# invictus717/MiCo

Hardware: AMD Instinct MI355X
Metric: omni-modal samples/sec (ViT-g/14 fwd+bwd) (higher is better)
Workload: dtype fp16

## Files before the change

mico_amd/csrc/attention.hip:

```cpp
#include "common.h"
#include <type_traits>

namespace {

constexpr float NEG_BIG = -1.0e30f;

#ifndef MICO_ATTN_PRIO
#define MICO_ATTN_PRIO 0
#endif

#ifdef MICO_ATTN_PHASES
__device__ unsigned long long g_attn_phase[4096 * 8];
#define PH_DECL unsigned long long ph_t = __builtin_readcyclecounter(), ph_acc[8] = {0, 0, 0, 0, 0, 0, 0, 0}
#define PH(slot) do { const unsigned long long n_ = __builtin_readcyclecounter(); ph_acc[slot] += n_ - ph_t; ph_t = n_; } while (0)
#define PH_STORE do { const int wg_ = (blockIdx.z * gridDim.y + blockIdx.y) * gridDim.x + blockIdx.x; \
        if (lane == 0 && wave == 0 && wg_ < 4096) for (int e_ = 0; e_ < 8; ++e_) g_attn_phase[wg_ * 8 + e_] = ph_acc[e_]; } while (0)
#else
#define PH_DECL
#define PH(slot)
#define PH_STORE
#endif

template <int HDP> struct Cfg {
    static constexpr int RS = 256;
// ... 32 lines not shown
}
template <int HDP>
__device__ __forceinline__ void tile_commit(const s16x8 (&reg)[Cfg<HDP>::NCH], LDS_AS char* tile, const TileMap<HDP>& m) {
#pragma unroll
    for (int it = 0; it < Cfg<HDP>::NCH; ++it) *(LDS_AS s16x8*)(tile + m.loff[it]) = reg[it];
}

template <typename T, int HDP>
__device__ __forceinline__ void row_frags(s16x8 (&f)[Cfg<HDP>::KS], const T* base, int64_t rs, int row, int nrows, int hd,
                                          int lane) {
#pragma unroll
    for (int ks = 0; ks < Cfg<HDP>::KS; ++ks) {
        const int d = ks * 32 + (lane >> 4) * 8;
        s16x8 v = {0, 0, 0, 0, 0, 0, 0, 0};
        if (row < nrows && d < hd) v = *(const s16x8*)(base + (int64_t)row * rs + d);
        f[ks] = v;
    }
}

template <int KM> __device__ __forceinline__ int swz_key(int row) {
    return KM == 0 ? ((row & 7) << 1) : (((row & 3) << 2) | ((row >> 2) & 3));
}
template <int HDP, int KM = 0>
__device__ __forceinline__ s16x8 lds_row_frag(LDS_AS const char* tile, int r0, int ks, int lane) {
    const int row = r0 + (lane & 15), ch = ks * 4 + (lane >> 4);
    return *(LDS_AS const s16x8*)(tile + row * Cfg<HDP>::RS + ((ch ^ swz_key<KM>(row)) << 4));
}
template <int HDP, int KM = 0>
__device__ __forceinline__ s16x8 lds_tr_frag(LDS_AS const char* tile, int td, int s2, int lane) {
    const int g = lane >> 4, p = lane & 15;
    const int ch = td * 2 + ((p >> 1) & 1), half = (p & 1) * 8;
    const int r_lo = (2 * s2) * 16 + g * 4 + (p >> 2);
    const int col_b = ((ch ^ swz_key<KM>(r_lo)) << 4) + half;
    s16x4 lo = __builtin_amdgcn_ds_read_tr16_b64_v4i16((LDS_AS s16x4*)(tile + r_lo * Cfg<HDP>::RS + col_b));
    s16x4 hi = __builtin_amdgcn_ds_read_tr16_b64_v4i16((LDS_AS s16x4*)(tile + (r_lo + 16) * Cfg<HDP>::RS + col_b));
    s16x8 r;
    r[0] = lo[0]; r[1] = lo[1]; r[2] = lo[2]; r[3] = lo[3];
    r[4] = hi[0]; r[5] = hi[1]; r[6] = hi[2]; r[7] = hi[3];
    return r;
}

__device__ __forceinline__ void lds_dma16(__amdgpu_buffer_rsrc_t rsrc, unsigned lds_dst, unsigned voffset) {
    unsigned keep;
    const unsigned dst = __builtin_amdgcn_readfirstlane(lds_dst);
    asm volatile("s_mov_b32 %0, m0\n\ts_mov_b32 m0, %2\n\ts_nop 0\n\tbuffer_load_dwordx4 %1, %3, 0 offen lds\n\ts_mov_b32 m0, %0"
                 : "=&s"(keep) : "v"(voffset), "s"(dst), "s"(rsrc) : "memory");
}

__device__ __forceinline__ void* uniform_ptr(const void* ptr) {
    const unsigned long long v = (unsigned long long)ptr;
    const unsigned lo = __builtin_amdgcn_readfirstlane((unsigned)v), hi = __builtin_amdgcn_readfirstlane((unsigned)(v >> 32));
    return (void*)(((unsigned long long)hi << 32) | lo);
}

template <typename T>
__device__ __forceinline__ s16x8 pack_pair(const f32x4& a, const f32x4& b) {
    typename T16<T>::v8 v;
    v[0] = (T)a[0]; v[1] = (T)a[1]; v[2] = (T)a[2]; v[3] = (T)a[3];
    v[4] = (T)b[0]; v[5] = (T)b[1]; v[6] = (T)b[2]; v[7] = (T)b[3];
    return __builtin_bit_cast(s16x8, v);
}

__device__ __forceinline__ float group_max(float v) { return xor32_max(xor16_max(v)); }
__device__ __forceinline__ float group_sum(float v) { return xor32_sum(xor16_sum(v)); }

__device__ __forceinline__ float mask_val(const float* mask, int mode, int b, int i, int j, int Sq, int Sk) {
    if (mode == 1) return mask[(int64_t)b * Sk + j];
    if (mode == 2) return mask[((int64_t)b * Sq + i) * Sk + j];
    return 0.f;
}

template <typename T, int HDP, bool DROP, int RB, int NW = 4>
__global__ __launch_bounds__(NW * 64, 2) void attn_fwd_kernel(const T* __restrict__ q, const T* __restrict__ k,
                                                              const T* __restrict__ v, T* __restrict__ o,
                                                              float* __restrict__ lse, const mico_attn_params p) {
    using C = Cfg<HDP>;
    __shared__ __attribute__((aligned(16))) char smem[2 * C::TILE];
    LDS_AS char* kt = (LDS_AS char*)smem;
    LDS_AS char* vt = kt + C::TILE;
    const int tid = threadIdx.x, lane = tid & 63, wave = tid >> 6;
    const bool stager = NW == 4 || tid < 256;
    const int b = blockIdx.z, h = blockIdx.y, q0 = blockIdx.x * (NW * 16 * RB);
    const T* qb = q + (int64_t)b * p.q_bs + h * p.hd;
    const int kvb = p.kv_index ? p.kv_index[b] : (p.kv_batch_mod > 0 ? b % p.kv_batch_mod : b);
    const T* kb = k + (int64_t)kvb * p.k_bs + h * p.hd;
    const T* vb = v + (int64_t)kvb * p.v_bs + h * p.hd;
    const int i0 = q0 + wave * (16 * RB) + (lane & 15);
    const int g = lane >> 4;
    const bool wave_live = q0 + wave * (16 * RB) < p.Sq;

    s16x8 qf[RB][C::KS];
    f32x4 oacc[RB][C::TD];
    float m_run[RB], l_run[RB];
#pragma unroll
    for (int rb = 0; rb < RB; ++rb) {
        row_frags<T, HDP>(qf[rb], qb, p.q_rs, i0 + rb * 16, p.Sq, p.hd, lane);
#pragma unroll
        for (int t = 0; t < C::TD; ++t) oacc[rb][t] = (f32x4){0.f, 0.f, 0.f, 0.f};
        m_run[rb] = NEG_BIG;
        l_run[rb] = 0.f;
    }
    const float sc2 = p.scale * 1.4426950408889634f;

    const int nt = (p.Sk + 63) / 64;
    const TileMap<HDP> tm_a = tile_map<HDP>(p.k_rs, p.hd, tid), tm_b = tile_map<HDP>(p.v_rs, p.hd, tid);
    s16x8 kr[C::NCH], vr[C::NCH];
// ... 82 lines not shown
#pragma unroll
                    for (int tn = 0; tn < 4; ++tn)
#pragma unroll
                        for (int r = 0; r < 4; ++r)
                            s[rb][tn][r] *= drop_hash_t(h0, tb + (unsigned)(tn * 16 + r) * 0x85EBCA6Bu) >= thr ? ik : 0.f;
                } else {
#pragma unroll
                    for (int tn = 0; tn < 4; ++tn)
#pragma unroll
                        for (int r = 0; r < 4; ++r)
                            s[rb][tn][r] *= drop_mult(p.drop_seed, p.drop_site, rowbase + (t * 64 + tn * 16 + g * 4 + r), thr, ik);
                }
            }
            l_run[rb] = l_run[rb] * alpha + group_sum(lloc);
            m_run[rb] = m_new;
#pragma unroll
            for (int t2 = 0; t2 < C::TD; ++t2) oacc[rb][t2] *= alpha;
            pf[rb][0] = pack_pair<T>(s[rb][0], s[rb][1]);
            pf[rb][1] = pack_pair<T>(s[rb][2], s[rb][3]);
        }
        PH(5);
#pragma unroll
        for (int s2 = 0; s2 < 2; ++s2) {
            if (2 * s2 >= ntn || !wave_live) continue;
#pragma unroll
            for (int td = 0; td < C::TD; ++td) {
                const s16x8 a = lds_tr_frag<HDP>(vt, td, s2, lane);
#pragma unroll
                for (int rb = 0; rb < RB; ++rb) oacc[rb][td] = T16<T>::mfma(a, pf[rb][s2], oacc[rb][td]);
            }
        }
        PH(6);
    }
    PH_STORE;
#pragma unroll
    for (int rb = 0; rb < RB; ++rb) {
        const int i = i0 + rb * 16;
        if (i < p.Sq) {
            const float inv = 1.f / l_run[rb];
            T* ob = o + (int64_t)b * p.o_bs + (int64_t)i * p.o_rs + h * p.hd;
#pragma unroll
            for (int td = 0; td < C::TD; ++td) {
                const int d = td * 16 + g * 4;
                if (d < p.hd)
                    *(s16x4*)(ob + d) = pack4<T>(oacc[rb][td][0] * inv, oacc[rb][td][1] * inv, oacc[rb][td][2] * inv, oacc[rb][td][3] * inv);
            }
            if (g == 0) lse[((int64_t)b * p.H + h) * p.Sq + i] = (m_run[rb] + __log2f(l_run[rb])) * 0.6931471805599453f;
        }
    }
}

constexpr int RES_KR = 288;

template <typename T, int HDP, int RB, int NSUB, bool ALL>
__device__ __forceinline__ void res_tile_step(LDS_AS const char* ktile, LDS_AS const char* vtile, const int key0, const int lo,
                                              const int hi, const int mode, const s16x8 (&qf)[RB][Cfg<HDP>::KS],
                                              f32x4 (&oacc)[RB][Cfg<HDP>::TD], float (&m_run)[RB], float (&l_run)[RB],
                                              const int Sk, const float sc2, const int lane,
                                              const int (&rf)[Cfg<HDP>::KS], const int (&tf)[Cfg<HDP>::TD]) {
    using C = Cfg<HDP>;
    constexpr int NH = (NSUB + 1) / 2;
    const int g = lane >> 4;
    f32x4 s[RB][NH * 2];
    if (ALL) {
        s16x8 an[C::KS];
#pragma unroll
        for (int ks = 0; ks < C::KS; ++ks) an[ks] = *(LDS_AS const s16x8*)(ktile + rf[ks]);
#pragma unroll
        for (int tn = 0; tn < NH * 2; ++tn) {
#pragma unroll
            for (int rb = 0; rb < RB; ++rb) s[rb][tn] = (f32x4){0.f, 0.f, 0.f, 0.f};
            if (tn >= NSUB) continue;
            s16x8 ac[C::KS];
#pragma unroll
            for (int ks = 0; ks < C::KS; ++ks) ac[ks] = an[ks];
            if (tn + 1 < NSUB) {
#pragma unroll
                for (int ks = 0; ks < C::KS; ++ks) an[ks] = *(LDS_AS const s16x8*)(ktile + rf[ks] + (tn + 1) * 16 * C::RS);
            }
            __builtin_amdgcn_sched_barrier(0);
#pragma unroll
            for (int ks = 0; ks < C::KS; ++ks)
#pragma unroll
                for (int rb = 0; rb < RB; ++rb) s[rb][tn] = T16<T>::mfma(ac[ks], qf[rb][ks], s[rb][tn]);
            __builtin_amdgcn_sched_barrier(0);
        }
    } else {
#pragma unroll
        for (int tn = 0; tn < NH * 2; ++tn) {
#pragma unroll
            for (int rb = 0; rb < RB; ++rb) s[rb][tn] = (f32x4){0.f, 0.f, 0.f, 0.f};
            if (tn < NSUB && tn >= lo && tn < hi) {
#pragma unroll
                for (int ks = 0; ks < C::KS; ++ks) {
                    const s16x8 a = *(LDS_AS const s16x8*)(ktile + rf[ks] + tn * 16 * C::RS);
#pragma unroll
                    for (int rb = 0; rb < RB; ++rb) s[rb][tn] = T16<T>::mfma(a, qf[rb][ks], s[rb][tn]);
                }
            }
        }
    }
    s16x8 pf[RB][NH];
#pragma unroll
    for (int rb = 0; rb < RB; ++rb) {
        float mloc = NEG_BIG;
#pragma unroll
        for (int tn = 0; tn < NH * 2; ++tn) {
            if (tn >= NSUB) {
                s[rb][tn] = (f32x4){NEG_BIG, NEG_BIG, NEG_BIG, NEG_BIG};
            } else if (mode == 0 || (mode == 1 && tn < NSUB - 1)) {
                s[rb][tn] *= sc2;
                mloc = fmaxf(fmaxf(mloc, fmaxf(s[rb][tn][0], s[rb][tn][1])), fmaxf(s[rb][tn][2], s[rb][tn][3]));
            } else {
                const int lim = (ALL || (tn >= lo && tn < hi)) ? Sk - key0 - tn * 16 - g * 4 : 0;
#pragma unroll
                for (int r = 0; r < 4; ++r) {
                    const float x = r < lim ? s[rb][tn][r] * sc2 : NEG_BIG;
                    s[rb][tn][r] = x;
                    mloc = fmaxf(mloc, x);
                }
            }
        }
        const float m_new = fmaxf(m_run[rb], group_max(mloc));
        const float alpha = __builtin_amdgcn_exp2f(m_run[rb] - m_new);
        float lloc = 0.f;
#pragma unroll
        for (int tn = 0; tn < NH * 2; ++tn) {
            if (tn >= NSUB) {
                s[rb][tn] = (f32x4){0.f, 0.f, 0.f, 0.f};
            } else {
#pragma unroll
                for (int r = 0; r < 4; ++r) {
                    const float e = __builtin_amdgcn_exp2f(s[rb][tn][r] - m_new);
                    s[rb][tn][r] = e;
                    lloc += e;
                }
            }
        }
        l_run[rb] = l_run[rb] * alpha + group_sum(lloc);
        m_run[rb] = m_new;
#pragma unroll
        for (int t2 = 0; t2 < C::TD; ++t2) oacc[rb][t2] *= alpha;
#pragma unroll
        for (int s2 = 0; s2 < NH; ++s2) pf[rb][s2] = pack_pair<T>(s[rb][2 * s2], s[rb][2 * s2 + 1]);
    }
    auto vfrag = [&](int idx) -> s16x8 {
        const int s2 = idx / C::TD, td = idx - s2 * C::TD;
        const s16x4 alo = __builtin_amdgcn_ds_read_tr16_b64_v4i16((LDS_AS s16x4*)(vtile + tf[td] + s2 * 32 * C::RS));
        const s16x4 ahi = __builtin_amdgcn_ds_read_tr16_b64_v4i16((LDS_AS s16x4*)(vtile + tf[td] + s2 * 32 * C::RS + 16 * C::RS));
        return (s16x8){alo[0], alo[1], alo[2], alo[3], ahi[0], ahi[1], ahi[2], ahi[3]};
    };
    if (ALL) {
        constexpr int NF = NH * C::TD, AH = 3;
        s16x8 ring[AH];
#pragma unroll
        for (int i = 0; i < AH; ++i) ring[i] = vfrag(i);
#pragma unroll
        for (int i = 0; i < NF; ++i) {
            const s16x8 a = ring[i % AH];
            if (i + AH < NF) ring[i % AH] = vfrag(i + AH);
            __builtin_amdgcn_sched_barrier(0);
#pragma unroll
            for (int rb = 0; rb < RB; ++rb) oacc[rb][i % C::TD] = T16<T>::mfma(a, pf[rb][i / C::TD], oacc[rb][i % C::TD]);
            __builtin_amdgcn_sched_barrier(0);
        }
    } else {
#pragma unroll
        for (int s2 = 0; s2 < NH; ++s2) {
            if (2 * s2 + 1 < lo || 2 * s2 >= hi) continue;
#pragma unroll
            for (int td = 0; td < C::TD; ++td) {
                const s16x8 a = vfrag(s2 * C::TD + td);
#pragma unroll
                for (int rb = 0; rb < RB; ++rb) oacc[rb][td] = T16<T>::mfma(a, pf[rb][s2], oacc[rb][td]);
            }
        }
    }
}

#ifndef MICO_ATTN_R1
#define MICO_ATTN_R1 0
#endif
template <int HDP> struct ResCfg {
    static constexpr int NXMAX = HDP <= 96 ? 4 : 3;
    static constexpr int PST = HDP + 2;
};

template <typename T, int HDP>
__global__ __launch_bounds__(512, 1) void attn_fwd_res_kernel(const T* __restrict__ q, const T* __restrict__ k,
                                                              const T* __restrict__ v, T* __restrict__ o,
                                                              float* __restrict__ lse, const mico_attn_params p) {
    using C = Cfg<HDP>;
    using R = ResCfg<HDP>;
    constexpr int CPR = HDP / 8;
    constexpr int NLD = 256 * CPR / 512;
    __shared__ __attribute__((aligned(16))) char smem[2 * RES_KR * C::RS + 8 * R::NXMAX * R::PST * 4];
    LDS_AS char* kt = (LDS_AS char*)smem;
    LDS_AS char* vt = kt + RES_KR * C::RS;
    LDS_AS float* part = (LDS_AS float*)(vt + RES_KR * C::RS);
    const int tid = threadIdx.x, lane = tid & 63, wave = tid >> 6;
    const int g = lane >> 4;
    const float sc2 = p.scale * 1.4426950408889634f;
    const int nitems = p.B * p.H;

    for (int c = tid; c < 32 * 16; c += 512) {
        *(LDS_AS s16x8*)(kt + 256 * C::RS + c * 16) = (s16x8){0, 0, 0, 0, 0, 0, 0, 0};
        *(LDS_AS s16x8*)(vt + 256 * C::RS + c * 16) = (s16x8){0, 0, 0, 0, 0, 0, 0, 0};
    }
    const int xrow = 256 + tid / CPR, xch = tid - (tid / CPR) * CPR;
    const bool xlive = xrow < p.Sk && xch * 8 < p.hd;
    const int xoff = xrow * C::RS + ((xch ^ ((xrow & 7) << 1)) << 4);

    int rf[C::KS], tf[C::TD];
#pragma unroll
    for (int ks = 0; ks < C::KS; ++ks) rf[ks] = (lane & 15) * C::RS + (((ks * 4 + g) ^ ((lane & 7) << 1)) << 4);
    {
        const int pp = lane & 15, r8 = g * 4 + (pp >> 2);
#pragma unroll
        for (int td = 0; td < C::TD; ++td) tf[td] = r8 * C::RS + (((td * 2 + ((pp >> 1) & 1)) ^ ((r8 & 7) << 1)) << 4) + (pp & 1) * 8;
    }
    const int nst = (p.Sk + 15) >> 4;
    constexpr bool WIDE = HDP <= 64;
    const bool wide_last = WIDE && nst > 4 && (nst & 3) == 1;
    const bool r1 = MICO_ATTN_R1 && !WIDE && p.Sk > 64 && (p.Sk & 63) == 1;
    const int nstm = r1 ? nst - 1 : nst;
    const int nsteps = wide_last ? (nst >> 2) : ((nstm + 3) >> 2);
    const int nx = p.Sq - 256;
    const int xt = wave >> 1, xlo = (wave & 1) * 2;
    const int xhi = wave == 7 ? nst - 12 : min(xlo + 2, nst - 4 * xt);

    auto kv_off = [&](int it) -> unsigned {
        if (it == NLD) return xlive ? (unsigned)(xrow * p.k_rs * 2 + xch * 16) : 0xFFFFFFF0u;
        const int c = it * 512 + tid;
        const int row = c / CPR, ch = c - row * CPR;
        return (row < p.Sk && ch * 8 < p.hd) ? (unsigned)(row * p.k_rs * 2 + ch * 16) : 0xFFFFFFF0u;
    };
    const int kbytes = (int)(((int64_t)(p.Sk - 1) * p.k_rs + p.hd) * 2), vbytes = (int)(((int64_t)(p.Sk - 1) * p.v_rs + p.hd) * 2);
    const int qbytes = (int)(((int64_t)(p.Sq - 1) * p.q_rs + p.hd) * 2);
    auto q_off = [&](int rb, int ks) -> unsigned {
        const int row = (rb < 2 ? wave * 32 + rb * 16 : 256) + (lane & 15), d = ks * 32 + g * 8;
        return (row < p.Sq && d < p.hd) ? (unsigned)(row * p.q_rs * 2 + d * 2) : 0xFFFFFFF0u;
    };
    s16x8 kr[NLD + 1], vr[NLD + 1];
    auto prefetch_part = [&](int item, int part_id) {
        const int b = item / p.H, h = item - b * p.H;
        __amdgpu_buffer_rsrc_t rk = __builtin_amdgcn_make_buffer_rsrc((void*)(k + (int64_t)b * p.k_bs + h * p.hd), 0, kbytes, 0x00020000);
#pragma unroll
        for (int it = 0; it <= NLD; ++it) {
            if (it * 4 / (NLD + 1) != part_id) continue;
            kr[it] = __builtin_bit_cast(s16x8, __builtin_amdgcn_raw_buffer_load_b128(rk, kv_off(it), 0, 0));
        }
    };
    auto load_v = [&](int item) {
// ... 36 lines not shown
        }
    };
    const int nwg = gridDim.x;
    int item = (int)blockIdx.x;
    int item_step = nwg;
    if ((nwg & 7) == 0 && nitems % nwg == 0) {
        const int per_wg = nitems / nwg;
        item = ((int)(blockIdx.x & 7) * (nwg >> 3) + (int)(blockIdx.x >> 3)) * per_wg;
        item_step = 1;
    }
    const int item_end = item_step == 1 ? item + nitems / nwg : nitems;
    if (item < item_end) {
#pragma unroll
        for (int pt = 0; pt < 4; ++pt) prefetch_part(item, pt);
        load_v(item);
        load_q(item);
    }

    int prev = -1;
    PH_DECL;
    for (; item < item_end; item += item_step) {
        PH(7);
        const int b = item / p.H, h = item - b * p.H;
#if MICO_ATTN_PRIO
        if (((item ^ (wave >> 2)) & 1) != 0) __builtin_amdgcn_s_setprio(1); else __builtin_amdgcn_s_setprio(0);
#endif
        const int next = item + item_step < item_end ? item + item_step : item;
        __syncthreads();
        PH(0);
        if (nx > 0 && prev >= 0) merge(prev);
        PH(1);
#pragma unroll
        for (int it = 0; it < NLD; ++it) {
            const int c = it * 512 + tid;
            const int row = c / CPR, ch = c - row * CPR;
            const int off = row * C::RS + ((ch ^ ((row & 7) << 1)) << 4);
            *(LDS_AS s16x8*)(kt + off) = kr[it];
            *(LDS_AS s16x8*)(vt + off) = vr[it];
        }
        if (xlive) {
            *(LDS_AS s16x8*)(kt + xoff) = kr[NLD];
            *(LDS_AS s16x8*)(vt + xoff) = vr[NLD];
        }
        PH(2);
        __syncthreads();
        PH(3);
        prefetch_part(next, 0);
        PH(4);
        if (nx > 0) {
            f32x4 ox[1][C::TD];
            float mx[1] = {NEG_BIG}, lx[1] = {0.f};
#pragma unroll
            for (int t = 0; t < C::TD; ++t) ox[0][t] = (f32x4){0.f, 0.f, 0.f, 0.f};
            if (xhi > xlo)
                res_tile_step<T, HDP, 1, 5, false>(kt + xt * C::TILE, vt + xt * C::TILE, xt * 64, xlo, xhi, 2, qx, ox, mx, lx, p.Sk, sc2, lane, rf, tf);
            if ((lane & 15) < nx) {
                LDS_AS float* pr = part + (wave * R::NXMAX + (lane & 15)) * R::PST;
                if (g == 0) { pr[HDP] = mx[0]; pr[HDP + 1] = lx[0]; }
#pragma unroll
                for (int td = 0; td < C::TD; ++td)
#pragma unroll
                    for (int r = 0; r < 4; ++r) pr[td * 16 + g * 4 + r] = ox[0][td][r];
            }
        }
        prev = item;
        PH(5);
        const bool main_live = wave * 32 < p.Sq;
        const int i0 = wave * 32 + (lane & 15);
        f32x4 oacc[2][C::TD];
        float m_run[2] = {NEG_BIG, NEG_BIG}, l_run[2] = {0.f, 0.f};
#pragma unroll
        for (int t = 0; t < C::TD; ++t) {
            oacc[0][t] = (f32x4){0.f, 0.f, 0.f, 0.f};
            oacc[1][t] = (f32x4){0.f, 0.f, 0.f, 0.f};
        }
        if (r1 && main_live) {
            LDS_AS const char* krow = kt + (p.Sk - 1) * C::RS;
            LDS_AS const char* vrow = vt + (p.Sk - 1) * C::RS;
            float dot[2] = {0.f, 0.f};
#pragma unroll
            for (int ks = 0; ks < C::KS; ++ks) {
                float k8[8];
                unpack8<T>(*(LDS_AS const s16x8*)(krow + ((ks * 4 + g) << 4)), k8);
#pragma unroll
                for (int rb = 0; rb < 2; ++rb) {
                    float q8[8];
                    unpack8<T>(qf[rb][ks], q8);
#pragma unroll
                    for (int e = 0; e < 8; ++e) dot[rb] = __builtin_fmaf(q8[e], k8[e], dot[rb]);
                }
            }
#pragma unroll
            for (int rb = 0; rb < 2; ++rb) {
                m_run[rb] = group_sum(dot[rb]) * sc2;
                l_run[rb] = 1.f;
            }
#pragma unroll
            for (int td = 0; td < C::TD; ++td) {
                const f32x4 v4 = unpack4<T>(*(LDS_AS const s16x4*)(vrow + ((td * 2 + (g >> 1)) << 4) + (g & 1) * 8));
                oacc[0][td] = v4;
                oacc[1][td] = v4;
            }
        }
        auto key_step = [&](int t) {
            if (!main_live || t >= nsteps) return;
            LDS_AS const char* ktile = kt + t * C::TILE;
            LDS_AS const char* vtile = vt + t * C::TILE;
            if (WIDE && t == nsteps - 1 && wide_last) {
                res_tile_step<T, HDP, 2, 5, true>(ktile, vtile, t * 64, 0, 5, (p.Sk & 15) ? 1 : 0, qf, oacc, m_run, l_run, p.Sk, sc2, lane, rf, tf);
            } else {
                const int ntn = min(4, nstm - 4 * t);
                if (ntn == 4) res_tile_step<T, HDP, 2, 4, true>(ktile, vtile, t * 64, 0, 4, t * 64 + 64 <= p.Sk ? 0 : 1, qf, oacc, m_run, l_run, p.Sk, sc2, lane, rf, tf);
                else res_tile_step<T, HDP, 2, 4, false>(ktile, vtile, t * 64, 0, ntn, 2, qf, oacc, m_run, l_run, p.Sk, sc2, lane, rf, tf);
            }
        };
        key_step(0);
        prefetch_part(next, 1);
        key_step(1);
        prefetch_part(next, 2);
        key_step(2);
        prefetch_part(next, 3);
        key_step(3);
        key_step(4);
        load_v(next);
        load_q(next);
        PH(6);
        if (main_live) {
            static_assert(C::TD % 2 == 0, "tile pairs");
#pragma unroll
            for (int rb = 0; rb < 2; ++rb) {
                const int i = i0 + rb * 16;
                const float inv = 1.f / l_run[rb];
                T* ob = o + (int64_t)b * p.o_bs + (int64_t)i * p.o_rs + h * p.hd;
#pragma unroll
                for (int tp = 0; tp < C::TD; tp += 2) {
                    const f32x4 ta = oacc[rb][tp], tb = oacc[rb][tp + 1];
                    u32x2 a2 = {pack2_scaled<T>(ta[0], ta[1], inv), pack2_scaled<T>(ta[2], ta[3], inv)};
                    u32x2 c2 = {pack2_scaled<T>(tb[0], tb[1], inv), pack2_scaled<T>(tb[2], tb[3], inv)};
                    asm volatile("s_nop 1\n\tv_permlane16_swap_b32 %0, %1" : "+v"(a2[0]), "+v"(c2[0]));
                    asm volatile("s_nop 1\n\tv_permlane16_swap_b32 %0, %1" : "+v"(a2[1]), "+v"(c2[1]));
                    const int d = (tp + (g & 1)) * 16 + (g >> 1) * 8;
                    if (i < p.Sq && d < p.hd) *(u32x4*)(ob + d) = (u32x4){a2[0], a2[1], c2[0], c2[1]};
                }
                if (i < p.Sq && g == 0) lse[((int64_t)b * p.H + h) * p.Sq + i] = (m_run[rb] + __log2f(l_run[rb])) * 0.6931471805599453f;
            }
        }
    }
    if (nx > 0 && prev >= 0) {
        __syncthreads();
        merge(prev);
    }
#ifdef MICO_ATTN_PHASES
    if (lane == 0 && blockIdx.x < 512) for (int e_ = 0; e_ < 8; ++e_) g_attn_phase[(blockIdx.x * 8 + wave) * 8 + e_] = ph_acc[e_];
#endif
}

template <typename T, int HDP, bool DROP>
__global__ __launch_bounds__(256, 2) void attn_bwd_dq_kernel(const T* __restrict__ q, const T* __restrict__ k,
                                                             const T* __restrict__ v, const T* __restrict__ o,
                                                             const T* __restrict__ d_o, const float* __restrict__ lse,
                                                             T* __restrict__ dq, float* __restrict__ delta,
                                                             const mico_attn_params p) {
    using C = Cfg<HDP>;
    __shared__ __attribute__((aligned(16))) char smem[2 * C::TILE];
    LDS_AS char* kt = (LDS_AS char*)smem;
    LDS_AS char* vt = kt + C::TILE;
    const int tid = threadIdx.x, lane = tid & 63, wave = tid >> 6;
    const int b = blockIdx.z, h = blockIdx.y, q0 = blockIdx.x * 64;
    const T* qb = q + (int64_t)b * p.q_bs + h * p.hd;
    const int kvb = p.kv_batch_mod > 0 ? b % p.kv_batch_mod : b;
    const T* kb = k + (int64_t)kvb * p.k_bs + h * p.hd;
    const T* vb = v + (int64_t)kvb * p.v_bs + h * p.hd;
    const T* ob = o + (int64_t)b * p.o_bs + h * p.hd;
    const T* dob = d_o + (int64_t)b * p.o_bs + h * p.hd;
    const int i = q0 + wave * 16 + (lane & 15);
    const int g = lane >> 4;
// ... 1353 lines not shown
            }
        }
        __syncthreads();
        __builtin_amdgcn_sched_barrier(0);
#pragma unroll
        for (int st = 0; st < 4; ++st) {
            if ((rd * 4 + st) * 32 >= p.Sk) continue;
            LDS_AS const char* skt = strips + st * S::WAVE;
            LDS_AS const char* sdst = skt + S::KT;
            if (wave < nti) {
                const s16x8 dsf = lds_tr_frag<64, 0>(sdst, wave, 0, lane);
#pragma unroll
                for (int td = 0; td < 4; ++td) dqw[td] = T16<T>::mfma(sq_tr_frag(skt, td, 0, lane), dsf, dqw[td]);
            }
            if (nti == 5) dq4 = T16<T>::mfma(sq_tr_frag(skt, wave, 0, lane), lds_tr_frag<64, 0>(sdst, 4, 0, lane), dq4);
        }
        __syncthreads();
#pragma unroll
        for (int kbk = 0; kbk < 2; ++kbk)
#pragma unroll
            for (int ks = 0; ks < 2; ++ks) {
                kf[kbk][ks] = nkf[kbk][ks];
                vf[kbk][ks] = nvf[kbk][ks];
            }
    }

    {
        const int i = wave * 16 + (lane & 15);
        if (i < p.Sq) {
            T* dqb = dq + (int64_t)b * p.q_bs + (int64_t)i * p.q_rs + h * HD;
#pragma unroll
            for (int td = 0; td < 4; ++td) *(s16x4*)(dqb + td * 16 + g * 4) = pack4<T>(dqw[td][0], dqw[td][1], dqw[td][2], dqw[td][3]);
        }
        const int i4 = 64 + (lane & 15);
        if (i4 < p.Sq)
            *(s16x4*)(dq + (int64_t)b * p.q_bs + (int64_t)i4 * p.q_rs + h * HD + wave * 16 + g * 4) = pack4<T>(dq4[0], dq4[1], dq4[2], dq4[3]);
    }
}

template <int HDP> struct OpCfg {
    using C = Cfg<HDP>;
    static constexpr int NST = 3;
    static constexpr int QT = 32 * C::RS;
    static constexpr int STAGE = 2 * QT;
    static constexpr int KROWS = 272;
    static constexpr int KT = KROWS * C::RS;
    static constexpr int DSK = 32 * 64;
    static constexpr int DSB = 8 * DSK;
    static constexpr int SST = 96;
    static constexpr int STAT = NST * SST * 4;
    static constexpr int X16 = 8 * 2 * HDP * 4;
    static constexpr int LDS = KT + NST * STAGE + 2 * DSB + STAT + X16;
};
__device__ __forceinline__ int launder(int x) { asm volatile("" : "+v"(x)); return x; }
__device__ __forceinline__ int ds_off(int kl, int qt, int pc) { return kl * 64 + ((((qt << 1) | (pc >> 1)) ^ ((kl >> 2) & 3)) << 4) + (pc & 1) * 8; }

template <typename T, int HDP, int KMODE>
__global__ __launch_bounds__(512, 1) void attn_bwd_onepass_kernel(const T* __restrict__ q, const T* __restrict__ k, const T* __restrict__ v,
                                                                  const T* __restrict__ o, const T* __restrict__ d_o, const float* __restrict__ lse,
                                                                  T* __restrict__ dq, T* __restrict__ dk, T* __restrict__ dv, const mico_attn_params p) {
    using C = Cfg<HDP>;
    using O = OpCfg<HDP>;
    constexpr int CPR = HDP / 8;
    __shared__ __attribute__((aligned(16))) char smem[O::LDS];
    LDS_AS char* kimg = (LDS_AS char*)smem;
    LDS_AS char* ring = kimg + O::KT;
    LDS_AS char* dsb = ring + O::NST * O::STAGE;
    LDS_AS float* stat = (LDS_AS float*)(dsb + 2 * O::DSB);
    LDS_AS float* x16 = stat + O::NST * O::SST;
    const int tid = threadIdx.x, lane = tid & 63, wave = __builtin_amdgcn_readfirstlane(tid >> 6), g = lane >> 4, l15 = lane & 15;
    constexpr float LOG2E = 1.4426950408889634f;
    const float sc2 = p.scale * LOG2E;
    const f32x4 zero4 = {0.f, 0.f, 0.f, 0.f};
    const s16x8 zero8 = {0, 0, 0, 0, 0, 0, 0, 0};
    const int nitems = p.B * p.H;
    const int NC = (p.Sq + 31) >> 5;
    const int nks = KMODE == 2 ? 9 : (KMODE == 1 ? 8 : (p.Sk + 31) >> 5);
    constexpr bool has16 = KMODE == 2, FULLK = KMODE != 0;
    const int dq_td = wave < 4 ? wave : 4 + ((wave - 4) >> 1);
    const int dq_qt = wave < 4 ? -1 : (wave & 1);

    const int nwg = gridDim.x;
    int item0 = (int)blockIdx.x, item_step = nwg, n_my = (nitems - (int)blockIdx.x + nwg - 1) / nwg;
    if ((nwg & 7) == 0 && nitems % nwg == 0) {
        n_my = nitems / nwg;
        item0 = ((int)(blockIdx.x & 7) * (nwg >> 3) + (int)(blockIdx.x >> 3)) * n_my;
        item_step = 1;
    }
    const int total = n_my * NC;

    for (int c = tid; c < 2 * O::DSB / 16; c += 512) *(LDS_AS s16x8*)(dsb + c * 16) = zero8;

    struct Piece { s16x8 o; float l; };
    const int lrow = tid >> 4, lch = (tid & 15) ^ (((tid >> 4) & 7) << 1), ach = tid & 15;
    const bool lch_ok = lch * 8 < p.hd, ach_ok = ach * 8 < p.hd;
    const int qbytes = (int)(((int64_t)(p.Sq - 1) * p.q_rs + p.hd) * 2), obytes = (int)(((int64_t)(p.Sq - 1) * p.o_rs + p.hd) * 2);
    int pf_c = 0, pf_left = n_my - 1, pf_b = item0 / p.H, pf_h = item0 - (item0 / p.H) * p.H;
    const unsigned ring_u = (unsigned)(uintptr_t)ring + (unsigned)(wave * 4 * C::RS);
    auto issue = [&](Piece& pc, int stage) {
        const int t = launder(tid);
        const int row = pf_c * 32 + (t >> 4);
        const bool rl = pf_left >= 0 && row < p.Sq, rp = rl && lch_ok, ra = rl && ach_ok;
        __amdgpu_buffer_rsrc_t rq = __builtin_amdgcn_make_buffer_rsrc((void*)(q + (int64_t)pf_b * p.q_bs + pf_h * p.hd), 0, qbytes, 0x00020000);
        __amdgpu_buffer_rsrc_t rd = __builtin_amdgcn_make_buffer_rsrc((void*)(d_o + (int64_t)pf_b * p.o_bs + pf_h * p.hd), 0, obytes, 0x00020000);
        __amdgpu_buffer_rsrc_t ro = __builtin_amdgcn_make_buffer_rsrc((void*)(o + (int64_t)pf_b * p.o_bs + pf_h * p.hd), 0, obytes, 0x00020000);
        __amdgpu_buffer_rsrc_t rs = __builtin_amdgcn_make_buffer_rsrc((void*)(lse + ((int64_t)pf_b * p.H + pf_h) * p.Sq), 0, p.Sq * 4, 0x00020000);
        const unsigned qo = rp ? (unsigned)(row * p.q_rs * 2 + lch * 16) : 0xFFFFFFF0u, oo = rp ? (unsigned)(row * p.o_rs * 2 + lch * 16) : 0xFFFFFFF0u;
        lds_dma16(rq, ring_u + stage * O::STAGE, qo);
        lds_dma16(rd, ring_u + stage * O::STAGE + O::QT, oo);
        pc.o = __builtin_bit_cast(s16x8, __builtin_amdgcn_raw_buffer_load_b128(ro, ra ? (unsigned)(row * p.o_rs * 2 + ach * 16) : 0xFFFFFFF0u, 0, 0));
        pc.l = __builtin_bit_cast(float, __builtin_amdgcn_raw_buffer_load_b32(rs, rl ? (unsigned)(row * 4) : 0xFFFFFFF0u, 0, 0));
        if (++pf_c == NC) {
            pf_c = 0;
            if (--pf_left >= 0) {
                pf_h += item_step;
                if (pf_h >= p.H) { const int nb = pf_h / p.H; pf_b += nb; pf_h -= nb * p.H; }
            }
        }
    };
    int cm_c = 0, cm_left = n_my - 1, cm_b = pf_b, cm_h = pf_h;
    s16x8 xk = zero8, xv = zero8;
    float dk8[8], dv8[8];
#pragma unroll
    for (int e = 0; e < 8; ++e) { dk8[e] = 0.f; dv8[e] = 0.f; }
    auto fetch256 = [&]() {
        if (KMODE != 2) return;
        const bool ok = cm_left >= 0 && ach_ok;
        __amdgpu_buffer_rsrc_t rk = __builtin_amdgcn_make_buffer_rsrc((void*)(k + (int64_t)cm_b * p.k_bs + cm_h * p.hd), 0, (int)(((int64_t)(p.Sk - 1) * p.k_rs + p.hd) * 2), 0x00020000);
        __amdgpu_buffer_rsrc_t rv = __builtin_amdgcn_make_buffer_rsrc((void*)(v + (int64_t)cm_b * p.v_bs + cm_h * p.hd), 0, (int)(((int64_t)(p.Sk - 1) * p.v_rs + p.hd) * 2), 0x00020000);
        xk = __builtin_bit_cast(s16x8, __builtin_amdgcn_raw_buffer_load_b128(rk, ok ? (unsigned)(256 * p.k_rs * 2 + ach * 16) : 0xFFFFFFF0u, 0, 0));
        xv = __builtin_bit_cast(s16x8, __builtin_amdgcn_raw_buffer_load_b128(rv, ok ? (unsigned)(256 * p.v_rs * 2 + ach * 16) : 0xFFFFFFF0u, 0, 0));
    };
    auto commit = [&](const Piece& pc, int stage) {
        int t = tid;
        asm volatile("" : "+v"(t) : "v"(pc.o));
        const int roff = (t >> 4) * C::RS + (((t & 15) ^ (((t >> 4) & 7) << 1)) << 4);
        const s16x8 dpc = *(LDS_AS const s16x8*)(ring + stage * O::STAGE + O::QT + roff);
        float a[8], c8[8], dl = 0.f;
        unpack8<T>(pc.o, a);
        unpack8<T>(dpc, c8);
#pragma unroll
        for (int e = 0; e < 8; ++e) dl += a[e] * c8[e];
        dl = row16_sum(dl) * p.scale;
        const float l2 = pc.l * LOG2E;
        LDS_AS float* ss = stat + stage * O::SST;
        if ((t & 15) == 0) { ss[32 + (t >> 4)] = dl; ss[t >> 4] = l2; }
        if (KMODE == 2) {
            const s16x8 qpc = *(LDS_AS const s16x8*)(ring + stage * O::STAGE + roff);
            float q8[8], k8[8], v8[8], sp = 0.f, dpp = 0.f;
            unpack8<T>(qpc, q8);
            unpack8<T>(xk, k8);
            unpack8<T>(xv, v8);
#pragma unroll
            for (int e = 0; e < 8; ++e) { sp += q8[e] * k8[e]; dpp += c8[e] * v8[e]; }
            sp = row16_sum(sp);
            dpp = row16_sum(dpp);
            const float pv = __builtin_amdgcn_exp2f(fmaf(sp, sc2, -l2));
            const float ds = pv * fmaf(dpp, p.scale, -dl);
#pragma unroll
            for (int e = 0; e < 8; ++e) { dk8[e] = fmaf(ds, q8[e], dk8[e]); dv8[e] = fmaf(pv, c8[e], dv8[e]); }
            if ((t & 15) == 1) ss[64 + (t >> 4)] = ds;
            if (++cm_c == NC) {
                cm_c = 0;
#pragma unroll
                for (int e = 0; e < 8; ++e) {
                    dk8[e] = group_sum(dk8[e]);
                    dv8[e] = group_sum(dv8[e]);
                }
                if (t < 16 + (t & ~63) && ach_ok) {
                    LDS_AS float* xw = x16 + wave * 2 * HDP + ach * 8;
                    *(LDS_AS f32x4*)xw = (f32x4){dk8[0], dk8[1], dk8[2], dk8[3]};
                    *(LDS_AS f32x4*)(xw + 4) = (f32x4){dk8[4], dk8[5], dk8[6], dk8[7]};
                    *(LDS_AS f32x4*)(xw + HDP) = (f32x4){dv8[0], dv8[1], dv8[2], dv8[3]};
// ... 517 lines not shown
```

Measured before the change: 43.82.

## Split residual attention tile step into score and PV phases, trim partial tiles

Splits the residual forward tile step into separate score/softmax and P·V helpers. It adds a variant that runs only the live 16-key subtiles (1 to 4) of a partial last tile or extra-row tile, instead of the masked lo/hi path that still walked the full loop. Inner tiles now always take the unmasked full path, and only the last tile handles ragged masking. The backward prefetch now tracks a flat item index with precomputed base offsets instead of incrementing batch/head, and the wave index is made wave-uniform with readfirstlane. The cost is extra template instantiations and more code size, which may affect register allocation.

```diff
diff --git a/mico_amd/csrc/attention.hip b/mico_amd/csrc/attention.hip
--- a/mico_amd/csrc/attention.hip
+++ b/mico_amd/csrc/attention.hip
@@ -108,6 +108,8 @@
     const unsigned lo = __builtin_amdgcn_readfirstlane((unsigned)v), hi = __builtin_amdgcn_readfirstlane((unsigned)(v >> 32));
     return (void*)(((unsigned long long)hi << 32) | lo);
 }
+
+__device__ __forceinline__ int launder(int x) { asm volatile("" : "+v"(x)); return x; }
 
 template <typename T>
 __device__ __forceinline__ s16x8 pack_pair(const f32x4& a, const f32x4& b) {
@@ -296,17 +298,16 @@
 
 constexpr int RES_KR = 288;
 
-template <typename T, int HDP, int RB, int NSUB, bool ALL>
-__device__ __forceinline__ void res_tile_step(LDS_AS const char* ktile, LDS_AS const char* vtile, const int key0, const int lo,
-                                              const int hi, const int mode, const s16x8 (&qf)[RB][Cfg<HDP>::KS],
-                                              f32x4 (&oacc)[RB][Cfg<HDP>::TD], float (&m_run)[RB], float (&l_run)[RB],
-                                              const int Sk, const float sc2, const int lane,
-                                              const int (&rf)[Cfg<HDP>::KS], const int (&tf)[Cfg<HDP>::TD]) {
+template <typename T, int HDP, int RB, int NSUB, int NHP>
+__device__ __forceinline__ void res_scores(LDS_AS const char* ktile, const int key0, const bool ragged, const s16x8 (&qf)[RB][Cfg<HDP>::KS],
+                                           float (&m_run)[RB], float (&l_run)[RB], s16x8 (&pf)[RB][NHP], float (&alpha)[RB],
+                                           const int Sk, const float sc2, const int lane, const int (&rf)[Cfg<HDP>::KS]) {
     using C = Cfg<HDP>;
     constexpr int NH = (NSUB + 1) / 2;
+    static_assert(NH <= NHP, "pf holds every half");
     const int g = lane >> 4;
     f32x4 s[RB][NH * 2];
-    if (ALL) {
+    {
         s16x8 an[C::KS];
 #pragma unroll
         for (int ks = 0; ks < C::KS; ++ks) an[ks] = *(LDS_AS const s16x8*)(ktile + rf[ks]);
@@ -329,34 +330,17 @@
                 for (int rb = 0; rb < RB; ++rb) s[rb][tn] = T16<T>::mfma(ac[ks], qf[rb][ks], s[rb][tn]);
             __builtin_amdgcn_sched_barrier(0);
         }
-    } else {
-#pragma unroll
-        for (int tn = 0; tn < NH * 2; ++tn) {
-#pragma unroll
-            for (int rb = 0; rb < RB; ++rb) s[rb][tn] = (f32x4){0.f, 0.f, 0.f, 0.f};
-            if (tn < NSUB && tn >= lo && tn < hi) {
-#pragma unroll
-                for (int ks = 0; ks < C::KS; ++ks) {
-                    const s16x8 a = *(LDS_AS const s16x8*)(ktile + rf[ks] + tn * 16 * C::RS);
-#pragma unroll
-                    for (int rb = 0; rb < RB; ++rb) s[rb][tn] = T16<T>::mfma(a, qf[rb][ks], s[rb][tn]);
-                }
-            }
-        }
-    }
-    s16x8 pf[RB][NH];
+    }
 #pragma unroll
     for (int rb = 0; rb < RB; ++rb) {
         float mloc = NEG_BIG;
 #pragma unroll
-        for (int tn = 0; tn < NH * 2; ++tn) {
-            if (tn >= NSUB) {
-                s[rb][tn] = (f32x4){NEG_BIG, NEG_BIG, NEG_BIG, NEG_BIG};
-            } else if (mode == 0 || (mode == 1 && tn < NSUB - 1)) {
+        for (int tn = 0; tn < NSUB; ++tn) {
+            if (!ragged || tn < NSUB - 1) {
                 s[rb][tn] *= sc2;
                 mloc = fmaxf(fmaxf(mloc, fmaxf(s[rb][tn][0], s[rb][tn][1])), fmaxf(s[rb][tn][2], s[rb][tn][3]));
             } else {
-                const int lim = (ALL || (tn >= lo && tn < hi)) ? Sk - key0 - tn * 16 - g * 4 : 0;
+                const int lim = launder(Sk - key0 - tn * 16 - g * 4);
 #pragma unroll
                 for (int r = 0; r < 4; ++r) {
                     const float x = r < lim ? s[rb][tn][r] * sc2 : NEG_BIG;
@@ -366,60 +350,84 @@
             }
         }
         const float m_new = fmaxf(m_run[rb], group_max(mloc));
-        const float alpha = __builtin_amdgcn_exp2f(m_run[rb] - m_new);
+        alpha[rb] = __builtin_amdgcn_exp2f(m_run[rb] - m_new);
         float lloc = 0.f;
 #pragma unroll
-        for (int tn = 0; tn < NH * 2; ++tn) {
-            if (tn >= NSUB) {
-                s[rb][tn] = (f32x4){0.f, 0.f, 0.f, 0.f};
-            } else {
-#pragma unroll
-                for (int r = 0; r < 4; ++r) {
-                    const float e = __builtin_amdgcn_exp2f(s[rb][tn][r] - m_new);
-                    s[rb][tn][r] = e;
-                    lloc += e;
-                }
-            }
-        }
-        l_run[rb] = l_run[rb] * alpha + group_sum(lloc);
+        for (int tn = 0; tn < NSUB; ++tn) {
+#pragma unroll
+            for (int r = 0; r < 4; ++r) {
+                const float e = __builtin_amdgcn_exp2f(s[rb][tn][r] - m_new);
+                s[rb][tn][r] = e;
+                lloc += e;
+            }
+        }
+        l_run[rb] = l_run[rb] * alpha[rb] + group_sum(lloc);
         m_run[rb] = m_new;
 #pragma unroll
-        for (int t2 = 0; t2 < C::TD; ++t2) oacc[rb][t2] *= alpha;
-#pragma unroll
-        for (int s2 = 0; s2 < NH; ++s2) pf[rb][s2] = pack_pair<T>(s[rb][2 * s2], s[rb][2 * s2 + 1]);
-    }
+        for (int s2 = 0; s2 < NHP; ++s2)
+            pf[rb][s2] = s2 < NH ? pack_pair<T>(s[rb][2 * s2], s[rb][2 * s2 + 1]) : (s16x8){0, 0, 0, 0, 0, 0, 0, 0};
+    }
+}
+template <typename T, int HDP, int RB, int NH, int NHP>
+__device__ __forceinline__ void res_pv(LDS_AS const char* vtile, const int h0, const s16x8 (&pf)[RB][NHP], f32x4 (&oacc)[RB][Cfg<HDP>::TD],
+                                       const int (&tf)[Cfg<HDP>::TD]) {
+    using C = Cfg<HDP>;
     auto vfrag = [&](int idx) -> s16x8 {
         const int s2 = idx / C::TD, td = idx - s2 * C::TD;
         const s16x4 alo = __builtin_amdgcn_ds_read_tr16_b64_v4i16((LDS_AS s16x4*)(vtile + tf[td] + s2 * 32 * C::RS));
         const s16x4 ahi = __builtin_amdgcn_ds_read_tr16_b64_v4i16((LDS_AS s16x4*)(vtile + tf[td] + s2 * 32 * C::RS + 16 * C::RS));
         return (s16x8){alo[0], alo[1], alo[2], alo[3], ahi[0], ahi[1], ahi[2], ahi[3]};
     };
-    if (ALL) {
-        constexpr int NF = NH * C::TD, AH = 3;
-        s16x8 ring[AH];
-#pragma unroll
-        for (int i = 0; i < AH; ++i) ring[i] = vfrag(i);
-#pragma unroll
-        for (int i = 0; i < NF; ++i) {
-            const s16x8 a = ring[i % AH];
-            if (i + AH < NF) ring[i % AH] = vfrag(i + AH);
-            __builtin_amdgcn_sched_barrier(0);
-#pragma unroll
-            for (int rb = 0; rb < RB; ++rb) oacc[rb][i % C::TD] = T16<T>::mfma(a, pf[rb][i / C::TD], oacc[rb][i % C::TD]);
-            __builtin_amdgcn_sched_barrier(0);
-        }
-    } else {
-#pragma unroll
-        for (int s2 = 0; s2 < NH; ++s2) {
-            if (2 * s2 + 1 < lo || 2 * s2 >= hi) continue;
-#pragma unroll
-            for (int td = 0; td < C::TD; ++td) {
-                const s16x8 a = vfrag(s2 * C::TD + td);
-#pragma unroll
-                for (int rb = 0; rb < RB; ++rb) oacc[rb][td] = T16<T>::mfma(a, pf[rb][s2], oacc[rb][td]);
-            }
-        }
-    }
+    constexpr int NF = NH * C::TD, AH = 3;
+    s16x8 ring[AH];
+#pragma unroll
+    for (int i = 0; i < AH; ++i) ring[i] = vfrag(i);
+#pragma unroll
+    for (int i = 0; i < NF; ++i) {
+        const s16x8 a = ring[i % AH];
+        if (i + AH < NF) ring[i % AH] = vfrag(i + AH);
+        __builtin_amdgcn_sched_barrier(0);
+#pragma unroll
+        for (int rb = 0; rb < RB; ++rb) oacc[rb][i % C::TD] = T16<T>::mfma(a, pf[rb][h0 + i / C::TD], oacc[rb][i % C::TD]);
+        __builtin_amdgcn_sched_barrier(0);
+    }
+}
+template <typename T, int HDP, int RB, int NSUB>
+__device__ __forceinline__ void res_tile_step(LDS_AS const char* ktile, LDS_AS const char* vtile, const int key0, const bool ragged,
+                                              const s16x8 (&qf)[RB][Cfg<HDP>::KS],
+                                              f32x4 (&oacc)[RB][Cfg<HDP>::TD], float (&m_run)[RB], float (&l_run)[RB],
+                                              const int Sk, const float sc2, const int lane,
+                                              const int (&rf)[Cfg<HDP>::KS], const int (&tf)[Cfg<HDP>::TD]) {
+    constexpr int NH = (NSUB + 1) / 2;
+    s16x8 pf[RB][NH];
+    float alpha[RB];
+    res_scores<T, HDP, RB, NSUB, NH>(ktile, key0, ragged, qf, m_run, l_run, pf, alpha, Sk, sc2, lane, rf);
+#pragma unroll
+    for (int rb = 0; rb < RB; ++rb)
+#pragma unroll
+        for (int t2 = 0; t2 < Cfg<HDP>::TD; ++t2) oacc[rb][t2] *= alpha[rb];
+    res_pv<T, HDP, RB, NH, NH>(vtile, 0, pf, oacc, tf);
+}
+template <typename T, int HDP, int RB, int NMAX>
+__device__ __forceinline__ void res_tile_step_n(const int n, LDS_AS const char* ktile, LDS_AS const char* vtile, const int key0, const bool ragged,
+                                                const s16x8 (&qf)[RB][Cfg<HDP>::KS],
+                                                f32x4 (&oacc)[RB][Cfg<HDP>::TD], float (&m_run)[RB], float (&l_run)[RB],
+                                                const int Sk, const float sc2, const int lane,
+                                                const int (&rf)[Cfg<HDP>::KS], const int (&tf)[Cfg<HDP>::TD]) {
+    using C = Cfg<HDP>;
+    static_assert(NMAX == 3 || NMAX == 4, "two halves");
+    s16x8 pf[RB][2];
+    float alpha[RB];
+    if (n == 1) res_scores<T, HDP, RB, 1, 2>(ktile, key0, ragged, qf, m_run, l_run, pf, alpha, Sk, sc2, lane, rf);
+    else if (n == 2) res_scores<T, HDP, RB, 2, 2>(ktile, key0, ragged, qf, m_run, l_run, pf, alpha, Sk, sc2, lane, rf);
+    else if (NMAX == 3 || n == 3) res_scores<T, HDP, RB, 3, 2>(ktile, key0, ragged, qf, m_run, l_run, pf, alpha, Sk, sc2, lane, rf);
+    else res_scores<T, HDP, RB, NMAX, 2>(ktile, key0, ragged, qf, m_run, l_run, pf, alpha, Sk, sc2, lane, rf);
+#pragma unroll
+    for (int rb = 0; rb < RB; ++rb)
+#pragma unroll
+        for (int t2 = 0; t2 < C::TD; ++t2) oacc[rb][t2] *= alpha[rb];
+    res_pv<T, HDP, RB, 1, 2>(vtile, 0, pf, oacc, tf);
+    if (n > 2) res_pv<T, HDP, RB, 1, 2>(vtile + 32 * C::RS, 1, pf, oacc, tf);
 }
 
 #ifndef MICO_ATTN_R1
@@ -442,7 +450,7 @@
     LDS_AS char* kt = (LDS_AS char*)smem;
     LDS_AS char* vt = kt + RES_KR * C::RS;
     LDS_AS float* part = (LDS_AS float*)(vt + RES_KR * C::RS);
-    const int tid = threadIdx.x, lane = tid & 63, wave = tid >> 6;
+    const int tid = threadIdx.x, lane = tid & 63, wave = __builtin_amdgcn_readfirstlane(tid >> 6);
     const int g = lane >> 4;
     const float sc2 = p.scale * 1.4426950408889634f;
     const int nitems = p.B * p.H;
@@ -585,8 +593,14 @@
             float mx[1] = {NEG_BIG}, lx[1] = {0.f};
 #pragma unroll
             for (int t = 0; t < C::TD; ++t) ox[0][t] = (f32x4){0.f, 0.f, 0.f, 0.f};
-            if (xhi > xlo)
-                res_tile_step<T, HDP, 1, 5, false>(kt + xt * C::TILE, vt + xt * C::TILE, xt * 64, xlo, xhi, 2, qx, ox, mx, lx, p.Sk, sc2, lane, rf, tf);
+            if (xhi > xlo) {
+                const int xo = xt * C::TILE + xlo * 16 * C::RS;
+                LDS_AS const char* kx = kt + xo;
+                LDS_AS const char* vx = vt + xo;
+                const int k0 = xt * 64 + xlo * 16, nsub = xhi - xlo;
+                const bool rag = k0 + nsub * 16 > p.Sk;
+                res_tile_step_n<T, HDP, 1, 3>(nsub, kx, vx, k0, rag, qx, ox, mx, lx, p.Sk, sc2, lane, rf, tf);
+            }
             if ((lane & 15) < nx) {
                 LDS_AS float* pr = part + (wave * R::NXMAX + (lane & 15)) * R::PST;
                 if (g == 0) { pr[HDP] = mx[0]; pr[HDP + 1] = lx[0]; }
@@ -635,26 +649,32 @@
                 oacc[1][td] = v4;
             }
         }
-        auto key_step = [&](int t) {
-            if (!main_live || t >= nsteps) return;
-            LDS_AS const char* ktile = kt + t * C::TILE;
-            LDS_AS const char* vtile = vt + t * C::TILE;
-            if (WIDE && t == nsteps - 1 && wide_last) {
-                res_tile_step<T, HDP, 2, 5, true>(ktile, vtile, t * 64, 0, 5, (p.Sk & 15) ? 1 : 0, qf, oacc, m_run, l_run, p.Sk, sc2, lane, rf, tf);
-            } else {
-                const int ntn = min(4, nstm - 4 * t);
-                if (ntn == 4) res_tile_step<T, HDP, 2, 4, true>(ktile, vtile, t * 64, 0, 4, t * 64 + 64 <= p.Sk ? 0 : 1, qf, oacc, m_run, l_run, p.Sk, sc2, lane, rf, tf);
-                else res_tile_step<T, HDP, 2, 4, false>(ktile, vtile, t * 64, 0, ntn, 2, qf, oacc, m_run, l_run, p.Sk, sc2, lane, rf, tf);
-            }
+        auto inner_step = [&](int t) {
+            if (!main_live || t >= nsteps - 1) return;
+            res_tile_step<T, HDP, 2, 4>(kt + t * C::TILE, vt + t * C::TILE, t * 64, false, qf, oacc, m_run, l_run, p.Sk, sc2, lane, rf, tf);
         };
-        key_step(0);
+        auto last_step = [&]() {
+            if (!main_live) return;
+            const int t = nsteps - 1;
+            const int to = t * C::TILE;
+            LDS_AS const char* ktile = kt + to;
+            LDS_AS const char* vtile = vt + to;
+            if (WIDE && wide_last) {
+                res_tile_step<T, HDP, 2, 5>(ktile, vtile, t * 64, (p.Sk & 15) != 0, qf, oacc, m_run, l_run, p.Sk, sc2, lane, rf, tf);
+                return;
+            }
+            const int ntn = nstm - 4 * t;
+            const bool rag = t * 64 + ntn * 16 > p.Sk;
+            res_tile_step_n<T, HDP, 2, 4>(ntn, ktile, vtile, t * 64, rag, qf, oacc, m_run, l_run, p.Sk, sc2, lane, rf, tf);
+        };
+        inner_step(0);
         prefetch_part(next, 1);
-        key_step(1);
+        inner_step(1);
         prefetch_part(next, 2);
-        key_step(2);
+        inner_step(2);
         prefetch_part(next, 3);
-        key_step(3);
-        key_step(4);
+        inner_step(3);
+        last_step();
         load_v(next);
         load_q(next);
         PH(6);
@@ -2114,7 +2134,6 @@
     static constexpr int X16 = 8 * 2 * HDP * 4;
     static constexpr int LDS = KT + NST * STAGE + 2 * DSB + STAT + X16;
 };
-__device__ __forceinline__ int launder(int x) { asm volatile("" : "+v"(x)); return x; }
 __device__ __forceinline__ int ds_off(int kl, int qt, int pc) { return kl * 64 + ((((qt << 1) | (pc >> 1)) ^ ((kl >> 2) & 3)) << 4) + (pc & 1) * 8; }
 
 template <typename T, int HDP, int KMODE>
@@ -2157,16 +2176,23 @@
     const int lrow = tid >> 4, lch = (tid & 15) ^ (((tid >> 4) & 7) << 1), ach = tid & 15;
     const bool lch_ok = lch * 8 < p.hd, ach_ok = ach * 8 < p.hd;
     const int qbytes = (int)(((int64_t)(p.Sq - 1) * p.q_rs + p.hd) * 2), obytes = (int)(((int64_t)(p.Sq - 1) * p.o_rs + p.hd) * 2);
-    int pf_c = 0, pf_left = n_my - 1, pf_b = item0 / p.H, pf_h = item0 - (item0 / p.H) * p.H;
+    int pf_c = 0, pf_left = n_my - 1, pf_item = item0;
+    int64_t pf_qo = 0, pf_oo = 0;
+    auto pf_offsets = [&]() {
+        const int fb = pf_item / p.H, fh = pf_item - fb * p.H;
+        pf_qo = (int64_t)fb * p.q_bs + fh * p.hd;
+        pf_oo = (int64_t)fb * p.o_bs + fh * p.hd;
+    };
+    pf_offsets();
     const unsigned ring_u = (unsigned)(uintptr_t)ring + (unsigned)(wave * 4 * C::RS);
     auto issue = [&](Piece& pc, int stage) {
         const int t = launder(tid);
         const int row = pf_c * 32 + (t >> 4);
         const bool rl = pf_left >= 0 && row < p.Sq, rp = rl && lch_ok, ra = rl && ach_ok;
-        __amdgpu_buffer_rsrc_t rq = __builtin_amdgcn_make_buffer_rsrc((void*)(q + (int64_t)pf_b * p.q_bs + pf_h * p.hd), 0, qbytes, 0x00020000);
-        __amdgpu_buffer_rsrc_t rd = __builtin_amdgcn_make_buffer_rsrc((void*)(d_o + (int64_t)pf_b * p.o_bs + pf_h * p.hd), 0, obytes, 0x00020000);
-        __amdgpu_buffer_rsrc_t ro = __builtin_amdgcn_make_buffer_rsrc((void*)(o + (int64_t)pf_b * p.o_bs + pf_h * p.hd), 0, obytes, 0x00020000);
-        __amdgpu_buffer_rsrc_t rs = __builtin_amdgcn_make_buffer_rsrc((void*)(lse + ((int64_t)pf_b * p.H + pf_h) * p.Sq), 0, p.Sq * 4, 0x00020000);
+        __amdgpu_buffer_rsrc_t rq = __builtin_amdgcn_make_buffer_rsrc((void*)(q + pf_qo), 0, qbytes, 0x00020000);
+        __amdgpu_buffer_rsrc_t rd = __builtin_amdgcn_make_buffer_rsrc((void*)(d_o + pf_oo), 0, obytes, 0x00020000);
+        __amdgpu_buffer_rsrc_t ro = __builtin_amdgcn_make_buffer_rsrc((void*)(o + pf_oo), 0, obytes, 0x00020000);
+        __amdgpu_buffer_rsrc_t rs = __builtin_amdgcn_make_buffer_rsrc((void*)(lse + (int64_t)pf_item * p.Sq), 0, p.Sq * 4, 0x00020000);
         const unsigned qo = rp ? (unsigned)(row * p.q_rs * 2 + lch * 16) : 0xFFFFFFF0u, oo = rp ? (unsigned)(row * p.o_rs * 2 + lch * 16) : 0xFFFFFFF0u;
         lds_dma16(rq, ring_u + stage * O::STAGE, qo);
         lds_dma16(rd, ring_u + stage * O::STAGE + O::QT, oo);
@@ -2175,12 +2201,12 @@
         if (++pf_c == NC) {
             pf_c = 0;
             if (--pf_left >= 0) {
-                pf_h += item_step;
-                if (pf_h >= p.H) { const int nb = pf_h / p.H; pf_b += nb; pf_h -= nb * p.H; }
+                pf_item += item_step;
+                pf_offsets();
             }
         }
     };
-    int cm_c = 0, cm_left = n_my - 1, cm_b = pf_b, cm_h = pf_h;
+    int cm_c = 0, cm_left = n_my - 1, cm_b = item0 / p.H, cm_h = item0 - (item0 / p.H) * p.H;
     s16x8 xk = zero8, xv = zero8;
     float dk8[8], dv8[8];
 #pragma unroll
```

Result: no change. 43.98, median of 6 (+0.4%).
